# bolcom/serenade

Hardware: AMD Instinct MI355X
Metric: predict_next queries/sec (higher is better)
Workload: dtype u32 ids / i32 accumulators / f64 scores; 1 GPU; BASELINE configs[2]: synthetic 60000000 interactions / 1760000 items, k=1500 m=2500 idf_weighting=2 last_items=4 how_many=21; batch_per_gpu=1048576, query_pool_batches=2, parallelism=query-sharded replicas x1 (no data-path collective), index=csr (built by this library)

## Files before the change

serenade_amd/csrc/srn_fast.hip:

```cpp
#include <hip/hip_runtime.h>

#include <cstdio>
#include <cstdlib>

#include "srn_device.h"
#include "srn_prep.h"
#include "srn_kernels.h"

namespace srn {

#ifndef SRN_FAST_NT
#define SRN_FAST_NT 1
#endif
typedef uint32_t fin_v4u __attribute__((ext_vector_type(4)));
__device__ __forceinline__ void fin_store(uint4* p, const uint4& v) {
#if SRN_FAST_NT
    __builtin_nontemporal_store((fin_v4u{v.x, v.y, v.z, v.w}), reinterpret_cast<fin_v4u*>(p));
#else
    *p = v;
#endif
}
__device__ __forceinline__ uint4 fin_load(const uint4* p) {
#if SRN_FAST_NT
    const fin_v4u v = __builtin_nontemporal_load(reinterpret_cast<const fin_v4u*>(p)); return make_uint4(v.x, v.y, v.z, v.w);
#else
    return *p;
#endif
}
template <typename T> __device__ __forceinline__ void row_store(T* p, T v) {
#if SRN_FAST_NT
    __builtin_nontemporal_store(v, p);
#else
    *p = v;
#endif
}

enum { FS_NB = 0, FS_FAIL, FS_SURV, FS_CCNT, FS_HITS, FS_LIVE, FS_SCAN_A = 8, FS_SCAN_B = 8, FS_W3 = 8, FS_CLS = 16, FS_TACC = 32 };
static constexpr uint32_t F_SIDF = F_LDS_BYTES, F_SATTR = F_SIDF + 512 * 8, F_TOTAL = F_SATTR + 512, F_SINV = F_W10 + 384;
static_assert(F_TOTAL * F_WG_PER_CU <= 160 * 1024, "LDS budget with the sample constants");

#ifndef SRN_FAST_RELOAD_ROWS
#define SRN_FAST_RELOAD_ROWS 0
#endif
#ifndef SRN_FAST_PRIO_LEVELS
#define SRN_FAST_PRIO_LEVELS 22201333
#endif
enum { FP_REC = 10000000, FP_FRONT = 1000000, FP_CUT = 100000, FP_REQ = 10000, FP_WALK = 1000, FP_HARV = 100, FP_WB = 10, FP_HAND = 1 };
#ifndef SRN_FAST_PRIO_X
#define SRN_FAST_PRIO_X 92
#endif
#define FAST_PRIO_X(div) do { if (SRN_FAST_PRIO_LEVELS && ((SRN_FAST_PRIO_X) / (div)) % 10 != 9) __builtin_amdgcn_s_setprio((short)(((SRN_FAST_PRIO_X) / (div)) % 10)); } while (0)
#ifndef SRN_MID_PRIO_LEVELS
#define SRN_MID_PRIO_LEVELS SRN_FAST_PRIO_LEVELS
#endif
#define FAST_PRIO(ph) do { if (SRN_FAST_PRIO_LEVELS) __builtin_amdgcn_s_setprio((short)((((MID) ? (SRN_MID_PRIO_LEVELS) : (SRN_FAST_PRIO_LEVELS)) / (ph)) % 10)); } while (0)
#ifndef SRN_FAST_STOP
#define SRN_FAST_STOP (-1)
#endif
#ifndef SRN_FAST_TICK_TID
#define SRN_FAST_TICK_TID 0
#endif
#define FAST_TICK(ph) \
    do { if (ticking && tid == (SRN_FAST_TICK_TID)) { const long long t_ = clock64(); tacc[ph] += (unsigned long long)(t_ - t_prev); t_prev = t_; } } while (0); \
    if (SRN_FAST_STOP == (ph)) continue

__device__ __forceinline__ uint32_t fast_offset_of(uint32_t idx, uint64_t r) {
    if (idx < F_REP_ITEMS) return (F_DIRECT + idx * F_REP + ((uint32_t)r & (F_REP - 1u))) * 4u;
    return idx < F_DIRECT ? idx * 4u : (F_SKETCH - F_HOT) + (idx & (F_SK_WORDS - 1u)) * 4u;
}
#ifndef SRN_FAST_PHANTOM_OOR
#define SRN_FAST_PHANTOM_OOR 1
#endif
static constexpr uint32_t F_PHANTOM_WORDS = 256u;
static constexpr uint32_t F_PHANTOM = SRN_FAST_PHANTOM_OOR ? F_BIG_TOTAL - (F_TOTAL - F_SIDF) - 256u * 4u - F_M_MAX : F_DUMP;
static_assert(!SRN_FAST_PHANTOM_OOR || (F_PHANTOM >= F_TOTAL && F_PHANTOM % 4u == 0u), "the phantom words lie beyond the 53 KB forms' LDS allocation");
static_assert(F_PHANTOM + F_PHANTOM_WORDS * 4u - F_HOT <= 65536u, "16-bit row offsets");
static_assert(!SRN_FAST_PHANTOM_OOR || F_PHANTOM_WORDS * 4u <= F_M_MAX, "inside the numerator bytes' room");
__device__ __forceinline__ uint32_t fast_phantom(uint64_t r, uint32_t j) {
    return (F_PHANTOM - F_HOT) + ((((uint32_t)r * 0x9E3779B1u + j * 0x85EBCA6Bu) >> 21) & (F_PHANTOM_WORDS - 1u)) * 4u;
}
__global__ __launch_bounds__(1024) void rows_to_packed_kernel(const uint64_t* __restrict__ row_off, const uint32_t* __restrict__ row_items, uint64_t n,
                                                              const uint32_t* __restrict__ block_base, uint32_t* __restrict__ packed, uint32_t* __restrict__ ext16) {
    __shared__ uint32_t wave_tot[16];
    const uint64_t r = (uint64_t)blockIdx.x * 1024 + threadIdx.x;
    const int lane = threadIdx.x & 63, wave = threadIdx.x >> 6;
    uint64_t o = 0, len = 0;
    if (r < n) { o = row_off[r]; len = row_off[r + 1] - o; }
    const uint32_t e = len > 30 ? (uint32_t)((len - 28 + 7) / 8) : 0u;
    const uint32_t inc = wave_incl_scan(e);
    if (lane == 63) wave_tot[wave] = inc;
    __syncthreads();
    uint32_t base = block_base[blockIdx.x];
    for (int w = 0; w < wave; ++w) base += wave_tot[w];
    const uint32_t eblk = base + inc - e;
    if (r > n) return;
    const uint32_t inl = len > 30 ? 28u : (uint32_t)len;
    uint32_t sl[16];
    auto half = [&](uint32_t j) -> uint32_t { return j < inl ? fast_offset_of(row_items[o + j], r) : fast_phantom(r, j); };
    sl[0] = (uint32_t)(len > 0xFFFFu ? 0xFFFFu : len);
#pragma unroll
    for (uint32_t wd = 1; wd < 16; ++wd) sl[wd] = half(2 * wd - 2) | (half(2 * wd - 1) << 16);
    if (len > 30) {
        sl[15] = eblk;
        for (uint32_t b = 0; b < e; ++b) {
            uint32_t wv[4];
#pragma unroll
            for (uint32_t x = 0; x < 4; ++x) {
                const uint64_t j0 = 28 + 8ull * b + 2 * x;
                const uint32_t lo = j0 < len ? fast_offset_of(row_items[o + j0], r) : fast_phantom(r, (uint32_t)j0);
                const uint32_t hi = j0 + 1 < len ? fast_offset_of(row_items[o + j0 + 1], r) : fast_phantom(r, (uint32_t)j0 + 1);
                wv[x] = lo | (hi << 16);
            }
            reinterpret_cast<uint4*>(ext16)[(size_t)eblk + b] = make_uint4(wv[0], wv[1], wv[2], wv[3]);
        }
    }
    uint4* dst = reinterpret_cast<uint4*>(packed + r * 16);
#pragma unroll
// ... 213 lines not shown
        if (f.serve == nullptr) {
        if (alen) { if (tid < 8u) a_items[tid] = f.tiny_items[tid]; if (tid == 0u) { a_off[0] = 0u; a_off[1] = alen; } __syncthreads(); }
        if (tid < PREP_LANES) prep_group(ix_arg, alen ? (const uint64_t*)a_items : p.items_flat, alen ? (const uint32_t*)a_off : p.q_off, alen ? 0u : blockIdx.x, tid, p.m, p.max_len,
                                         const_cast<char*>(p.prep) + (size_t)blockIdx.x * p.prep_stride, nullptr, 0u, nullptr);
        __syncthreads();
        }
    }

    uint32_t* misc = (uint32_t*)(smem + F_MISC);
    uint8_t* wlut = (uint8_t*)(smem + F_WLUT);
    uint16_t* w10t = (uint16_t*)(smem + F_W10);
    uint32_t* nbl = (uint32_t*)(smem + F_NBL);
    unsigned long long* ckey = (unsigned long long*)(smem + F_CAND);
    uint32_t* cidx = (uint32_t*)(smem + F_CAND + F_CAND_CAP * 8);
    char* const acc_base = smem + F_HOT;
    uint32_t* hot = (uint32_t*)(smem + F_HOT);
    uint32_t* ikeys = (uint32_t*)(smem + F_TABLE);
    int* iacc = (int*)(smem + F_TABLE + F_TABLE_WORDS * 4);
    uint2* hits = (uint2*)(smem + F_HITS);
    uint32_t* surv = (uint32_t*)(smem + F_SURV);
    constexpr uint32_t SURV_CAP = F_SURV_WORDS - 256u;
    uint32_t* const cls_area = BIG ? (uint32_t*)(smem + SIDF) - 256 : surv + SURV_CAP;
    uint32_t* const dn_area = cls_area - F_M_MAX / 4u;
    uint2* const nb2 = reinterpret_cast<uint2*>(dn_area - F_K_MAX * 2u);
    uint32_t* thist = surv + SURV_CAP;
    auto num_of = [&](uint32_t set) -> uint32_t {
        if constexpr (MID) return (uint32_t)wlut[set & 31u] + (uint32_t)wlut[32u + (set >> 5)];
        else return (uint32_t)wlut[set]; };
    auto w10_of = [&](uint32_t set) -> uint32_t {
        if constexpr (MID) { const uint32_t lo = set & 31u, hi = set >> 5; const uint32_t mp = lo ? (uint32_t)wlut[64u + lo] : (uint32_t)wlut[96u + hi]; return (9u - mp) * ((uint32_t)wlut[lo] + (uint32_t)wlut[32u + hi]); }
        else return (uint32_t)w10t[set]; };

    unsigned long long* tacc = (unsigned long long*)(smem + F_MISC + FS_TACC * 4);
    if (tid < 16u) tacc[tid] = 0ull;
    const bool ticking = p.phase_cycles != nullptr;
    const bool business = (p.flags & SRN_FLAG_BUSINESS_LOGIC) != 0u;
    const uint32_t n_kept = ix.n_kept;
    auto qpos = [&](uint32_t pq) -> uint32_t { return ((wave + NW * (pq >> 6)) << 6) + (pq & 63u); };

    uint32_t* const pre = (uint32_t*)(smem + F_W10 + 64);
    bool have_pre = false;
    { const ItemMeta m0 = f.meta_sample[tid];
      ((double*)(smem + SIDF))[tid] = m0.idf > 0.0 ? m0.idf : 1.0; ((uint8_t*)(smem + SATTR))[tid] = (uint8_t)m0.attr;
      if (tid < 16u) ((double*)(smem + SINV))[tid] = tid < 8u ? f.inv_idf_hot[tid] : f.inv_idf_hi; }
    const bool listed = !MID && MODE == FM_BACK && f.mid_list != nullptr;
    const uint32_t q_end = TINY ? p.nq : LONG ? *f.long_cnt : BIG ? *f.bigq_cnt : MID || listed ? *f.mid_cnt : p.nq;
    const bool ordered = !MID && MODE != FM_FRONT && f.order != nullptr && !listed;
    const uint32_t ox = blockIdx.x & 7u;
    const bool serving = TINY && f.serve != nullptr;
    const uint32_t qi_step = serving ? 0u : ordered ? gridDim.x >> 3 : gridDim.x;
    uint32_t serve_seq = 0u; bool serve_have = false; unsigned long long serve_t0 = 0ull, serve_c0 = 0ull;
    if constexpr (TINY) { if (serving) serve_seq = __atomic_load_n(&(f.serve + blockIdx.x)->done_seq, __ATOMIC_RELAXED); }
    const uint32_t qi_end = ordered ? ord_count(f.order_dups != nullptr ? p.nq - *f.order_dups : p.nq, ox) : q_end;
    for (uint32_t qi = ordered ? blockIdx.x >> 3 : (MODE == FM_FRONT ? f.q_base : 0u) + blockIdx.x; qi < qi_end; qi += qi_step) {
        if constexpr (TINY) {
            if (serving) {
                uint32_t* const sv_flag = reinterpret_cast<uint32_t*>(smem + F_W10 + 64 + 192);
                unsigned long long* const sv_items = reinterpret_cast<unsigned long long*>(smem + F_W10 + 64); uint32_t* const sv_off = reinterpret_cast<uint32_t*>(smem + F_W10 + 64 + 128);
                ServeCtl* const c = f.serve + blockIdx.x;
                __syncthreads();
                if (wave == 0u) {
                    __threadfence_system();
                    uint32_t leave = 0u;
                    if (serve_have && lane == 0u) {
                        const uint32_t cnt = __atomic_load_n(&p.out_counts[blockIdx.x], __ATOMIC_RELAXED);
                        if (cnt & 0x80000000u) { (void)atomicExch(&f.slow_cnt[SC_GENERAL], 0u); (void)atomicExch(&f.slow_cnt[SC_MID], 0u); (void)atomicExch(&f.slow_cnt[SC_BIG_TICKET_LO], 0u); (void)atomicExch(&f.slow_cnt[SC_BIG_TICKET_HI], 0u); }
                        const unsigned long long t_end = wall_clock64();
                        c->stamp[2] = (uint32_t)(t_end - serve_t0); c->stamp[3] = (uint32_t)((unsigned long long)clock64() - serve_c0);
                        __atomic_store_n(&c->count, cnt, __ATOMIC_RELAXED);
                        __atomic_store_n(&c->status, (cnt & 0x80000000u) ? 1u : 0u, __ATOMIC_RELAXED);
                        __threadfence_system();
                        __atomic_store_n(&c->done_seq, serve_seq, __ATOMIC_RELAXED);
                    }
                    const unsigned long long t0 = wall_clock64(), idle = __builtin_nontemporal_load(&c->idle_ticks);
                    uint32_t w = 0u, s_new = 0u, n = 0u;
                    for (;;) {
                        if (lane < 16u) w = __atomic_load_n(reinterpret_cast<const uint32_t*>(c) + lane, __ATOMIC_RELAXED);
                        s_new = (uint32_t)__builtin_amdgcn_readlane((int)w, 0); n = min((uint32_t)__builtin_amdgcn_readlane((int)w, 1), 16u);
                        if (s_new != serve_seq) {
                            uint32_t x = lane >= 4u && lane < 4u + 2u * min(n, 5u) ? w : 0u;
#pragma unroll
                            for (int d = 1; d < 16; d <<= 1) x ^= __shfl_xor(x, d, 16);
                            if ((uint32_t)__builtin_amdgcn_readlane((int)x, 0) == ((uint32_t)__builtin_amdgcn_readlane((int)w, 2) ^ s_new ^ n)) break;
                        }
                        if ((uint32_t)__builtin_amdgcn_readlane((int)w, 3) != 0u || wall_clock64() - t0 > idle) { leave = 1u; break; }
                    }
                    if (!leave) {
                        serve_seq = s_new; serve_have = true; serve_t0 = wall_clock64(); serve_c0 = (unsigned long long)clock64();
                        if (lane >= 4u && lane < 14u) reinterpret_cast<uint32_t*>(sv_items)[lane - 4u] = w;
                        if (n > 5u && lane < 2u * (n - 5u)) reinterpret_cast<uint32_t*>(sv_items)[10u + lane] = __atomic_load_n(reinterpret_cast<const uint32_t*>(c->more) + lane, __ATOMIC_RELAXED);
                        if (lane == 0u) { sv_off[0] = 0u; sv_off[1] = n; p.out_counts[blockIdx.x] = 0x80000002u; c->stamp[0] = (uint32_t)(serve_t0 - t0); }
                    }
                    if (lane == 0u) sv_flag[0] = leave;
                }
                __syncthreads();
                if (sv_flag[0] != 0u) break;
                if (tid < PREP_LANES) prep_group(ix_arg, (const uint64_t*)sv_items, (const uint32_t*)sv_off, 0u, tid, p.m, p.max_len, const_cast<char*>(p.prep) + (size_t)blockIdx.x * p.prep_stride, nullptr, 0u, nullptr);
                __syncthreads();
                if (tid == 0u) c->stamp[1] = (uint32_t)(wall_clock64() - serve_t0);
            }
        }
        const uint32_t q = TINY ? qi : LONG ? f.long_list[qi] : BIG ? f.bigq_list[qi] : MID || listed ? f.mid_list[qi] : ordered ? (uint32_t)f.order[ord_pos(ox, qi)] : qi;
        const uint32_t q_ord_next = ordered && qi + qi_step < qi_end ? (uint32_t)f.order[ord_pos(ox, qi + qi_step)]
                                  : listed && qi + qi_step < qi_end ? f.mid_list[qi + qi_step] : 0xFFFFFFFFu;
#ifndef SRN_MID_PREFETCH
#define SRN_MID_PREFETCH 0
#endif
        const uint32_t q_after = !(MID && SRN_MID_PREFETCH) ? 0xFFFFFFFFu : qi + gridDim.x < q_end ? (BIG ? f.bigq_list : f.mid_list)[qi + gridDim.x] : 0xFFFFFFFFu;
        long long t_prev = ticking ? clock64() : 0;
        FAST_PRIO(FP_REC);
        const char* const rec = p.prep + (size_t)q * p.prep_stride;
        struct { uint32_t U, rmax, xlo, sumw, L, n_staged, cur_attr, unsafe; } hd;
        constexpr uint32_t HW = (uint32_t)sizeof(PrepHead) / 4u;
        struct { uint32_t idx, kept; unsigned long long base; } x0{kNone, 0u, 0ull};
        if (have_pre) {
            auto uni = [&](uint32_t w) -> uint32_t { return (uint32_t)__builtin_amdgcn_readfirstlane((int)pre[w]); };
            hd.U = uni(0); hd.rmax = uni(1); hd.xlo = uni(2); hd.sumw = uni(3); hd.L = uni(6); hd.n_staged = uni(7); hd.cur_attr = uni(16); hd.unsafe = uni(17);
            if (lane < (LONG ? 32u : MID ? 16u : 8u) && lane < hd.L) { const uint32_t* it = pre + HW + 6u * lane; x0.idx = it[0]; x0.kept = it[3]; x0.base = ((unsigned long long)it[5] << 32) | it[4]; }
        } else {
            const PrepHead h0 = *(const PrepHead*)rec;
            hd.U = h0.U; hd.rmax = h0.rmax; hd.xlo = h0.xlo; hd.sumw = h0.sumw; hd.L = h0.L; hd.n_staged = h0.n_staged; hd.cur_attr = h0.cur_attr; hd.unsafe = h0.unsafe;
            if ((MID ? lane < (LONG ? 32u : 16u) && lane < p.max_len : lane < 8u) && lane < hd.L) { const PrepItem pi = ((const PrepItem*)(rec + sizeof(PrepHead)))[lane]; x0.idx = pi.idx; x0.kept = pi.kept; x0.base = pi.base; }
        }
        have_pre = false;
        const uint32_t L = hd.L, n = hd.n_staged, U = hd.U;
        unsigned long long rm = __ballot(x0.kept > 0u);
#ifdef SRN_FAST_EXP_ONELIST
        rm &= 0ull - rm;
#endif
        const uint32_t nr = (uint32_t)__popcll(rm);
        const bool rel = MID || (WIDE && nr > 3u);
        const uint32_t NB = LONG ? F_LONG_NB : MID ? max(nr, 4u) : WIDE && !rel ? 3u : 4u, NBM = (1u << NB) - 1u, base = rel ? hd.xlo : 0u;
        const bool fits = hd.unsafe != 0u ? false : LONG ? L >= 1u && L <= F_LONG_LMAX && L <= p.max_len && hd.sumw <= F_LONG_CLASSES && nr <= F_LONG_LISTS && 2u * n + 8u + F_LONG_RES_WORDS <= MW && hd.rmax - hd.xlo < (1u << (32u - F_LONG_NB))
                        : MID ? L >= 1u && L <= F_MID_LMAX && L <= p.max_len && hd.sumw <= F_MID_CLASSES && nr <= F_MID_LISTS && 2u * n + 8u + 256u <= MW && hd.rmax - hd.xlo < (1u << (32u - NB))
                              : L >= 1u && L <= 8u && L <= p.max_len && hd.sumw <= 15u && nr <= 4u && 2u * n + 8u <= MW && (!rel || hd.rmax - hd.xlo < (1u << 28));
        uint32_t* const xq = MODE == FM_FUSED ? nullptr : f.xchg + (size_t)q * f.xchg_stride;
        if (!fits) {
            if constexpr (MODE == FM_FRONT) { if (tid == 0) xq[0] = 0xFFFFFFFFu; }
            else if (tid == 0) {
                if (hd.unsafe != 0u) f.slow_list[atomicAdd(&f.slow_cnt[SC_GENERAL], 1u)] = q;
                else if (!MID && MODE == FM_FUSED && f.bigq_list != nullptr && L >= 1u && L <= 8u && L <= p.max_len && hd.sumw <= 15u && nr <= 4u && hd.rmax - hd.xlo < (1u << 28) &&
                    2u * n + 8u + 256u <= (F_BIG_TOTAL - (F_TOTAL - F_SIDF) - F_WORK) / 4u) f.bigq_list[atomicAdd(f.bigq_cnt, 1u)] = q;
                else if (!MID && MODE == FM_FUSED && f.mid_list != nullptr && L >= 1u && L <= F_MID_LMAX && L <= p.max_len) f.mid_list[atomicAdd(f.mid_cnt, 1u)] = q;
                else if (!MID && MODE == FM_FUSED && f.long_list != nullptr && L > F_MID_LMAX && L <= F_LONG_LMAX && L <= p.max_len) f.long_list[atomicAdd(f.long_cnt, 1u)] = q;
                else if (MID && !BIG && f.bigq_list != nullptr && L >= 1u && L <= F_MID_LMAX && L <= p.max_len && hd.sumw <= F_MID_CLASSES && nr <= F_MID_LISTS && hd.rmax - hd.xlo < (1u << (32u - NB)) &&
                         2u * n + 8u + 256u <= (F_BIG_TOTAL - (F_TOTAL - F_SIDF) - F_WORK) / 4u) f.bigq_list[atomicAdd(f.bigq_cnt, 1u)] = q;
                else f.slow_list[atomicAdd(&f.slow_cnt[SC_GENERAL], 1u)] = q;
            }
            continue;
        }
        if (n == 0u) { if (tid == 0) { if constexpr (MODE == FM_FRONT) xq[0] = 0u; else p.out_counts[q] = 0u; } continue; }
        uint32_t kp[NL], ps[NL]; const uint32_t* src[NL];
#pragma unroll
        for (int r = 0; r < NL; ++r) {
            const int l = rm ? __ffsll((long long)rm) - 1 : 0;
            kp[r] = rm ? (uint32_t)__builtin_amdgcn_readlane((int)x0.kept, l) : 0u;
            const uint32_t blo = (uint32_t)__builtin_amdgcn_readlane((int)(uint32_t)x0.base, l), bhi = (uint32_t)__builtin_amdgcn_readlane((int)(uint32_t)(x0.base >> 32), l);
            src[r] = ix.post_rank + (((unsigned long long)bhi << 32) | blo);
            ps[r] = (uint32_t)l;
            rm &= rm - 1ull;
        }
        const uint32_t cur_idx = (uint32_t)__builtin_amdgcn_readlane((int)x0.idx, 0);
        const uint32_t cur_attr = hd.cur_attr;
        const uint32_t s1 = kp[0], s2 = s1 + kp[1], s3 = s2 + kp[2];

        uint32_t v[4][5];
        uint32_t K = 0;
        uint32_t pfv[4] = {0u, 0u, 0u, 0u};
        uint32_t xsv[3] = {0u, 0u, 0u};
        if constexpr (MODE == FM_BACK) {
            const uint32_t kv = xq[0];
#pragma unroll
            for (int t = 0; t < 3; ++t) xsv[t] = xq[1u + min(wave * 64u + lane + (uint32_t)t * BLOCK, f.xchg_stride - 2u)];
            K = (uint32_t)__builtin_amdgcn_readfirstlane((int)kv);
        } else {
#pragma unroll
        for (int r = 0; r < 4; ++r)
#pragma unroll
            for (int j = 0; j < 5; ++j) { v[r][j] = 0u; if ((uint32_t)j * BLOCK < kp[r]) v[r][j] = src[r][min(tid + j * BLOCK, kp[r] - 1u)]; }
        }
        __syncthreads();
        FAST_PRIO(FP_FRONT);
        if constexpr (MODE != FM_BACK) {
#pragma unroll
        for (int r = 0; r < 4; ++r)
#pragma unroll
            for (int j = 0; j < 5; ++j) asm volatile("" : "+v"(v[r][j]));
        }
        FAST_TICK(0);
        if (tid < (uint32_t)FS_TACC) misc[tid] = 0;
#ifndef SRN_FAST_EARLY_CLEAR
#define SRN_FAST_EARLY_CLEAR 0
#endif
        const uint32_t clr_lo = (!SRN_FAST_EARLY_CLEAR || MODE == FM_FRONT) ? F_TABLE : (MODE == FM_BACK || nr <= 1u) ? F_HOT : min(F_TABLE, max(F_HOT, (F_WORK + (2u * n + 16u) * 4u + 15u) & ~15u));
        if (SRN_FAST_EARLY_CLEAR && MODE != FM_FRONT) {
            uint4* z = reinterpret_cast<uint4*>(smem);
            for (uint32_t i = clr_lo / 16u + tid; i < F_TABLE / 16u; i += BLOCK) z[i] = make_uint4(0u, 0u, 0u, 0u);
        }
        if constexpr (LONG) {
            if (tid < 32u) {
                uint32_t pr = 0u;
#pragma unroll
                for (int r = 0; r < NL; ++r) pr = tid == (uint32_t)(31 - r) ? ps[r] : pr;
                wlut[tid] = (uint8_t)(L - pr); wlut[32u + tid] = (uint8_t)pr;
            }
        } else
        if constexpr (MID) {
            if (tid < 64u) {
                const uint32_t half = tid >> 5, hs = tid & 31u;
                uint32_t num = 0u, mp = 0u;
                const uint32_t lo = hs ? (uint32_t)__ffs((int)hs) - 1u : 0u;
#pragma unroll
                for (int r = 0; r < 5; ++r) { const uint32_t pr = half ? ps[5 + r] : ps[r]; num += ((hs >> r) & 1u) ? L - pr : 0u; mp = lo == (uint32_t)r ? pr : mp; }
                wlut[tid] = (uint8_t)num; wlut[64u + tid] = (uint8_t)mp;
            }
        } else
        if (tid < (1u << nr)) {
            const uint32_t num = ((tid & 1u) ? L - ps[0] : 0u) + ((tid & 2u) ? L - ps[1] : 0u) + ((tid & 4u) ? L - ps[2] : 0u) + ((tid & 8u) ? L - ps[3] : 0u);
            const uint32_t lo = tid ? (uint32_t)__ffs((int)tid) - 1u : 0u;
            const uint32_t mp = lo == 0u ? ps[0] : lo == 1u ? ps[1] : lo == 2u ? ps[2] : ps[3];
            wlut[tid] = (uint8_t)num; w10t[tid] = (uint16_t)((9u - mp) * num);
        }
        if constexpr (MODE == FM_BACK) {
            if (K == 0xFFFFFFFFu) { if (tid == 0) f.slow_list[atomicAdd(&f.slow_cnt[SC_GENERAL], 1u)] = q; continue; }
            if (K == 0u) { if (tid == 0) p.out_counts[q] = 0u; continue; }
        } else
        if (nr == 1u) {
            K = min(kp[0], p.k);
#pragma unroll
            for (int j = 0; j < 3; ++j) { const uint32_t e = tid + j * BLOCK; if ((uint32_t)j * BLOCK < K && e < K) {
                if constexpr (LONG) nb2[e] = make_uint2(((v[0][j] - base) << NB) | 31u, (uint32_t)((9 - (int)ps[0]) * (int)(L - ps[0])));
                else nbl[e] = ((v[0][j] - base) << NB) | 1u; } }
            __syncthreads();
            FAST_TICK(1);
        } else {
        uint32_t* const B1 = (uint32_t*)(smem + F_WORK); uint32_t* const B0 = B1 + n;
        static_assert(F_WORK == F_NBL, "the m-cut writes the neighbour list in place");
        if constexpr (MID) {
            const uint32_t nlev = nr <= 2u ? 1u : nr <= 4u ? 2u : nr <= 8u ? 3u : nr <= 16u ? 4u : 5u;
            uint32_t* const X = (nlev & 1u) ? B1 : B0; uint32_t* const Y = (nlev & 1u) ? B0 : B1;
            uint32_t pre_r[NL];
// ... 199 lines not shown
        }
        }
        }

        FAST_TICK(4);
        if constexpr (SRN_FAST_ROW_PREFETCH == 2 && !MID && MODE == FM_FUSED && !FRAG) asm volatile("" :: "v"(pfv[0]), "v"(pfv[1]), "v"(pfv[2]), "v"(pfv[3]));
        FAST_PRIO(FP_REQ); FAST_PRIO_X(10);
        if constexpr (MODE == FM_FRONT) {
            if (tid == 0) xq[0] = K;
#pragma unroll
            for (int j = 0; j < 3; ++j) { const uint32_t e = tid + (uint32_t)j * BLOCK; if ((uint32_t)j * BLOCK < K && e < K) xq[1u + e] = nbl[e]; }
            continue;
        }

        uint32_t svr[3]; uint4 rq[3], rq1[3];
        uint32_t wvr[3] = {0u, 0u, 0u};
#pragma unroll
        for (int t = 0; t < 3; ++t) {
            const uint32_t j = wave * 64u + lane + (uint32_t)t * BLOCK;
            if constexpr (MODE == FM_BACK) svr[t] = j < K ? xsv[t] : 0u;
            else if constexpr (LONG) { const uint2 e2 = nb2[K ? min(j, K - 1u) : 0u]; svr[t] = K ? e2.x : 0u; wvr[t] = e2.y; }
            else
            svr[t] = K ? nbl[min(j, K - 1u)] : 0u;
            const size_t r = (MODE == FM_BACK ? j < K : K != 0u) ? (size_t)(base + (svr[t] >> NB)) : (size_t)n_kept;
            rq[t] = *reinterpret_cast<const uint4*>(&f.row_packed[r * (FRAG ? 1 : 4)]); rq1[t] = make_uint4(0u, 0u, 0u, 0u);
        }
        if (((SRN_FAST_PRIO_X) / 10) % 10 != 9) FAST_PRIO(FP_REQ);
        {
            uint4* z = reinterpret_cast<uint4*>(smem + F_HOT);
            for (uint32_t i = tid; i < (clr_lo - F_HOT) / 16u; i += BLOCK) z[i] = make_uint4(0u, 0u, 0u, 0u);
            if (tid < 64u) reinterpret_cast<uint4*>(thist)[tid] = make_uint4(0u, 0u, 0u, 0u);
            if (tid < F_TABLE_WORDS / 4u) { reinterpret_cast<uint4*>(ikeys)[tid] = make_uint4(EMPTY32, EMPTY32, EMPTY32, EMPTY32);
                                            reinterpret_cast<uint4*>(iacc)[tid] = make_uint4(0u, 0u, 0u, 0u); }
        }
        __syncthreads();
        FAST_PRIO(FP_WALK);
        FAST_TICK(8);
        auto add2 = [&](uint32_t wd, uint32_t w) {
            if constexpr (LONG) {
                const bool neg = (int)w < 0; const uint32_t a = wd & 0xFFFFu, b = wd >> 16;
                if (!neg || a < F_SKETCH - F_HOT) atomicAdd((uint32_t*)(acc_base + a), w);
                if (!neg || b < F_SKETCH - F_HOT) atomicAdd((uint32_t*)(acc_base + b), w);
            } else {
            atomicAdd((uint32_t*)(acc_base + (wd & 0xFFFFu)), w); atomicAdd((uint32_t*)(acc_base + (wd >> 16)), w); } };
        constexpr uint32_t INL1 = FRAG ? 6u : 14u, INL2 = FRAG ? 20u : 28u;
        uint32_t cnt3 = 0;
#pragma unroll
        for (int t = 0; t < 3; ++t) {
            const bool m3 = wave * 64u + lane + (uint32_t)t * BLOCK < K && (rq[t].x & 0xFFFFu) > INL1;
            const unsigned long long b3 = __ballot(m3);
            if (m3) nbl[qpos(cnt3 + (uint32_t)__popcll(b3 & lt))] = LONG ? wave * 64u + lane + (uint32_t)t * BLOCK : svr[t];
            cnt3 += (uint32_t)__popcll(b3);
        }
#ifdef SRN_FAST_SUBTICKS
        FAST_TICK(5);
#endif
        uint32_t wr[3];
#pragma unroll
        for (int t = 0; t < 3; ++t) wr[t] = LONG ? wvr[t] : w10_of(svr[t] & NBM);
        if constexpr (!FRAG) {
#pragma unroll
            for (int t = 0; t < 3; ++t) {
                const bool more6 = wave * 64u + lane + (uint32_t)t * BLOCK < K && (rq[t].x & 0xFFFFu) > 6u;
                const size_t r1 = more6 ? (size_t)(base + (svr[t] >> NB)) : (size_t)n_kept;
                rq1[t] = *reinterpret_cast<const uint4*>(&f.row_packed[r1 * 4 + 1]);
            }
        }
        auto tok_slot = [&](uint32_t tok) -> uint32_t { if constexpr (LONG) return nb2[tok].x; else return tok; };
        auto tok_w = [&](uint32_t tok, uint32_t slot) -> uint32_t { if constexpr (LONG) return nb2[tok].y; else return w10_of(slot & NBM); };
        auto q3_load = [&](uint32_t p0, uint32_t& tok, uint32_t& sv, uint32_t& hdr, uint4& c4, uint4& d4, uint32_t& blk) {
            tok = nbl[qpos(min(p0 + lane, cnt3 - 1u))];
            sv = tok_slot(tok);
            if constexpr (FRAG) {
                const uint4 s4 = *reinterpret_cast<const uint4*>(f.row_packed + (size_t)(base + (sv >> NB)));
                hdr = s4.x;
                const uint4* eb = reinterpret_cast<const uint4*>(f.row_ext16) + ((hdr & 0xFFFFu) > 6u ? (size_t)s4.w : (size_t)0);
                c4 = eb[0]; d4 = eb[1]; blk = s4.w + 2u;
            } else {
                const RowQuad* rowp = f.row_packed + (size_t)(base + (sv >> NB)) * 4;
                hdr = *reinterpret_cast<const uint32_t*>(rowp); c4 = *reinterpret_cast<const uint4*>(rowp + 2); d4 = *reinterpret_cast<const uint4*>(rowp + 3); blk = 0u;
            } };
        uint32_t tk3 = 0, sv3 = 0, hdr3 = 0, blk3 = 0; uint4 c43 = make_uint4(0u, 0u, 0u, 0u), d43 = c43;
        if (cnt3) q3_load(0u, tk3, sv3, hdr3, c43, d43, blk3);
        const uint32_t w3 = cnt3 ? tok_w(tk3, sv3) : 0u;
        const uint32_t qn = MID ? q_after : ordered || listed ? q_ord_next : q + gridDim.x;
        const bool park = MID ? q_after != 0xFFFFFFFFu : ordered || listed ? q_ord_next != 0xFFFFFFFFu : qn < p.nq;
        if (wave == 1u && park) {
            const char* const rn = p.prep + (size_t)qn * p.prep_stride + lane * 4u;
            const uint32_t dst = (uint32_t)__builtin_amdgcn_readfirstlane((int)lds_addr(pre));
            if (lane * 4u < p.prep_stride) glds_dword_uncounted(rn, dst);
            if (256u + lane * 4u < min(p.prep_stride, 320u)) glds_dword_uncounted(rn + 256, dst + 256u);
        }
#pragma unroll
        for (int t = 0; t < 3; ++t) {
            if (wave * 64u + (uint32_t)t * BLOCK < K) {
                const bool act = wave * 64u + lane + (uint32_t)t * BLOCK < K;
                const uint32_t w = wr[t], len = rq[t].x & 0xFFFFu;
                if constexpr (FRAG) { if (act) { add2(rq[t].y, w); add2(rq[t].z, w); if (len <= 6u) add2(rq[t].w, w); } }
                else if (act) { add2(rq[t].y, w); add2(rq[t].z, w); add2(rq[t].w, w); }
            }
        }
        if constexpr (!FRAG) {
#pragma unroll
        for (int t = 0; t < 3; ++t) {
            if (wave * 64u + (uint32_t)t * BLOCK < K) {
                const bool act = wave * 64u + lane + (uint32_t)t * BLOCK < K;
                const uint32_t w = wr[t], len = rq[t].x & 0xFFFFu;
                if (act && len > 6u) { add2(rq1[t].x, w); add2(rq1[t].y, w); add2(rq1[t].z, w); add2(rq1[t].w, w); }
            }
        }
        }
        auto add_tail = [&](uint32_t p0, uint32_t w, uint32_t hdr, const uint4& c4, const uint4& d4, uint32_t blk) {
            const bool act = p0 + lane < cnt3;
            const uint32_t len = hdr & 0xFFFFu;
            const bool more = FRAG ? true : len > 30u;
            if constexpr (FRAG) {
                if (act) { add2(c4.x, w); add2(c4.y, w); add2(c4.z, w); add2(c4.w, w); }
                if (act && len > 12u) { add2(d4.x, w); add2(d4.y, w); add2(d4.z, w); add2(d4.w, w); }
            } else if (act) {
                add2(c4.x, w); add2(c4.y, w); add2(c4.z, w); add2(c4.w, w);
                add2(d4.x, w); add2(d4.y, w); add2(d4.z, w);
                if (len <= 30u) add2(d4.w, w);
            }
            for (uint32_t t8 = INL2; __ballot(act && more && t8 < len) != 0ull; t8 += 8u) {
                if (act && more && t8 < len) {
                    const uint4 e4 = reinterpret_cast<const uint4*>(f.row_ext16)[(size_t)blk + ((t8 - INL2) >> 3)];
                    add2(e4.x, w); add2(e4.y, w); add2(e4.z, w); add2(e4.w, w);
                }
            } };
#ifdef SRN_FAST_SUBTICKS
        FAST_TICK(6);
#endif
        FAST_PRIO_X(1);
        { fin_v4u dv = {d43.x, d43.y, d43.z, d43.w};
          asm volatile("" : "+v"(hdr3), "+v"(dv));
          d43 = make_uint4(dv.x, dv.y, dv.z, dv.w); }
        if constexpr (!FRAG) blk3 = d43.w;
        if (cnt3) add_tail(0u, w3, hdr3, c43, d43, blk3);
        for (uint32_t p0 = 64u; p0 < cnt3; p0 += 64u) { uint32_t tk, sv, hdr, blk; uint4 c4, d4; q3_load(p0, tk, sv, hdr, c4, d4, blk); if constexpr (!FRAG) blk = d4.w; add_tail(p0, tok_w(tk, sv), hdr, c4, d4, blk); }
#ifdef SRN_FAST_SUBTICKS
        FAST_TICK(7);
#endif
        __syncthreads();
        FAST_PRIO(FP_HARV);
        FAST_TICK(9);
        uint32_t t32m1; uint32_t floor_b;
        {
            const uint32_t e = lane * NW + wave;
            uint32_t v = hot[e];
            if (F_REP_ITEMS && e < F_REP_ITEMS) {
                const uint4* rp = reinterpret_cast<const uint4*>(hot + F_DIRECT + e * F_REP);
                const uint4 a = rp[0], b = rp[1];
                v = a.x + a.y + a.z + a.w + b.x + b.y + b.z + b.w;
            }
            if (!SRN_FAST_PHANTOM_OOR || BIG)
            for (uint32_t i = tid; i < F_PHANTOM_WORDS; i += BLOCK) ((uint32_t*)(smem + F_PHANTOM))[i] = 0u;
            bool valid = (LONG ? (int)v > 0 : v != 0u) && e != cur_idx;
            double x = 0.0; uint32_t tie = 0;
            tie = f.meta_sample[tid].id_rank;
            if (business) valid = valid && business_ok(cur_attr, (uint32_t)((const uint8_t*)(smem + SATTR))[tid]);
            if (valid) x = ((const double*)(smem + SIDF))[tid] * (double)v;
            const uint32_t k32 = (uint32_t)((unsigned long long)__double_as_longlong(x) >> 32);
            {
                uint32_t vv = k32, third = 0;
#pragma unroll
                for (int t = 0; t < 3; ++t) {
                    const uint32_t mx = wave_max(vv);
                    third = mx;
                    const unsigned long long bal = __ballot(vv == mx);
                    if ((int)lane == __ffsll((long long)bal) - 1) vv = 0;
                }
                for (uint32_t t = 3u; t < ((p.how_many + 7u) >> 3); ++t) {
                    const uint32_t mx = wave_max(vv);
                    third = mx;
                    const unsigned long long bal = __ballot(vv == mx);
                    if ((int)lane == __ffsll((long long)bal) - 1) vv = 0;
                }
                if (lane == 0u) misc[FS_W3 + wave] = third;
            }
            __syncthreads();
            uint32_t t32 = 0xFFFFFFFFu;
#pragma unroll
            for (int w = 0; w < NW; ++w) t32 = min(t32, misc[FS_W3 + w]);
            t32m1 = t32 ? t32 - 1u : 0u;
            const bool take = valid && k32 >= t32m1;
            const uint32_t at = wave_append(take, &misc[FS_CCNT]);
            if (take) { if (at < F_CAND_CAP) { ckey[at] = (unsigned long long)__double_as_longlong(x); cidx[at] = tie; } else misc[FS_FAIL] = 1;
                        const uint32_t hb = k32 >> 16, tb = t32 >> 16; if (t32) atomicAdd(&thist[hb > tb ? min(hb - tb, 255u) : 0u], 1u); }
            const double x_lo = __longlong_as_double((long long)((unsigned long long)t32m1 << 32));
            const double inv = ((const double*)(smem + SINV))[min(lane, 8u)];
            const uint32_t my_floor = (uint32_t)fmin(4.0e9, fmax(1.0, floor(x_lo * inv * (1.0 - 1e-9)) - 1.0));
            floor_b = (uint32_t)__builtin_amdgcn_readlane((int)my_floor, 8);
            {
                const uint32_t wv = (uint32_t)__builtin_amdgcn_readfirstlane((int)wave);
                const uint4* h4 = reinterpret_cast<const uint4*>(hot);
                static_assert(F_HOT_WORDS == 4096 || F_HOT_WORDS == 3840, "quads per thread below (3840: the 40 KB timing experiment)");
                constexpr uint32_t NQ2 = F_HOT_WORDS / 4u - 128u - (uint32_t)BLOCK;
                const uint4 a4 = h4[128u + tid];
                const uint4 b4 = tid < NQ2 ? h4[128u + (uint32_t)BLOCK + tid] : make_uint4(0u, 0u, 0u, 0u);
                if (tid == NQ2 - 1u) hot[F_HOT_WORDS - 1u] = 0u;
                const uint32_t fl1 = (uint32_t)__builtin_amdgcn_readlane((int)my_floor, (int)(1u + (wv >> 1)));
                const uint32_t fl2 = (uint32_t)__builtin_amdgcn_readlane((int)my_floor, (int)min(5u + (wv >> 1), 7u));
                auto quad = [&](const uint4& q4, uint32_t e0, uint32_t fl) {
                    const uint32_t mx = LONG ? (uint32_t)max(max(max((int)q4.x, (int)q4.y), max((int)q4.z, (int)q4.w)), 0) : max(max(q4.x, q4.y), max(q4.z, q4.w));
                    if (__ballot(mx >= fl) == 0ull) return;
                    const uint32_t vv[4] = {q4.x, q4.y, q4.z, q4.w};
#pragma unroll
                    for (uint32_t j = 0; j < 4u; ++j) {
                        const uint32_t e2 = e0 + j;
                        const bool pass = (LONG ? (int)vv[j] >= (int)fl : vv[j] >= fl) && e2 != cur_idx && e2 < F_DIRECT;
                        const uint32_t at2 = wave_append(pass, &misc[FS_SURV]);
                        if (pass) { if (at2 < SURV_CAP && vv[j] < (1u << 20)) surv[at2] = (e2 << 20) | vv[j]; else atomicOr(&misc[FS_FAIL], 2u); }
                    } };
                quad(a4, 512u + 4u * tid, fl1);
                quad(b4, 512u + 4u * ((uint32_t)BLOCK + tid), fl2);
            }
        }
        __syncthreads();
        {
            const uint4 h4 = reinterpret_cast<const uint4*>(thist)[lane];
            const uint32_t sum4 = h4.x + h4.y + h4.z + h4.w, pre = wave_incl_scan(sum4);
            uint32_t above = (uint32_t)__builtin_amdgcn_readlane((int)pre, 63) - pre;
            const uint32_t need = p.how_many;
            const bool mine = above < need && need <= above + sum4;
            uint32_t bin = 4u * lane + 3u;
            if (above + h4.w < need) { above += h4.w; bin = 4u * lane + 2u;
                if (above + h4.z < need) { above += h4.z; bin = 4u * lane + 1u;
                    if (above + h4.y < need) bin = 4u * lane; } }
            const unsigned long long mb = __ballot(mine);
            const uint32_t bsel = mb ? (uint32_t)__builtin_amdgcn_readlane((int)bin, __ffsll((long long)mb) - 1) : 0u;
            if (bsel) {
                const uint32_t t32b = (((t32m1 + 1u) >> 16) + bsel) << 16;
                t32m1 = t32b - 1u;
// ... 6 lines not shown
        FAST_PRIO(FP_WB);
        {
            const uint32_t ns = min(misc[FS_SURV], SURV_CAP);
            for (uint32_t i = tid; i < ns; i += BLOCK) {
                const uint32_t sv = surv[i], e = sv >> 20, v = sv & 0xFFFFFu;
                const ItemMeta mt = ix.meta[e];
                const double x = (mt.idf > 0.0 ? mt.idf : 1.0) * (double)v;
                const bool take = (uint32_t)((unsigned long long)__double_as_longlong(x) >> 32) >= t32m1 && (!business || business_ok(cur_attr, mt.attr));
                const uint32_t at = wave_append(take, &misc[FS_CCNT]);
                if (take) { if (at < F_CAND_CAP) { ckey[at] = (unsigned long long)__double_as_longlong(x); cidx[at] = mt.id_rank; } else misc[FS_FAIL] = 1; }
            }
        }
        {
            const uint4* sk4 = reinterpret_cast<const uint4*>(smem + F_SKETCH);
            uint32_t mx = 0;
            for (uint32_t i = tid; i < F_SK_WORDS / 4u; i += BLOCK) { const uint4 w4 = sk4[i]; mx = max(max(mx, w4.x), max(max(w4.y, w4.z), w4.w)); }
            if (__ballot(mx >= floor_b) != 0ull && lane == 0u) misc[FS_LIVE] = 1u;
        }
        __syncthreads();
        have_pre = park;
        const bool live = misc[FS_LIVE] != 0u;
        if (live) {
        {
            uint32_t dbg_hits = 0;
            auto chk2 = [&](uint32_t hm, uint32_t wd) -> uint32_t {
                const uint32_t a = *(const uint32_t*)(acc_base + max(wd & 0xFFFFu, F_ZERO_OFF)), b = *(const uint32_t*)(acc_base + max(wd >> 16, F_ZERO_OFF));
                return (hm << 2) | (a >= floor_b ? 2u : 0u) | (b >= floor_b ? 1u : 0u); };
            auto list_hits = [&](uint32_t hm, uint32_t npos, uint32_t sv, uint32_t j0) {
                const uint32_t c = (uint32_t)__popc(hm);
                if (__ballot(c != 0u) == 0ull) return;
                dbg_hits += c;
                const uint32_t inc = wave_incl_scan(c);
                uint32_t base = 0; if (lane == 63u) base = atomicAdd(&misc[FS_HITS], inc);
                uint32_t at = (uint32_t)__builtin_amdgcn_readlane((int)base, 63) + inc - c;
                while (hm) {
                    const uint32_t b = 31u - (uint32_t)__clz((int)hm); hm &= ~(1u << b);
                    if (at < F_HIT_CAP) hits[at] = make_uint2(sv, j0 + (npos - 1u - b)); else atomicOr(&misc[FS_FAIL], 4u);
                    ++at;
                }
            };
            auto mx2 = [&](uint32_t mx, uint32_t wd) -> uint32_t {
                const uint32_t a = *(const uint32_t*)(acc_base + max(wd & 0xFFFFu, F_ZERO_OFF)), b = *(const uint32_t*)(acc_base + max(wd >> 16, F_ZERO_OFF));
                return max(max(mx, a), b); };
            uint32_t tk3b = 0, sv3b = 0, hdr3b = 0, blk3b = 0; uint4 c43b = make_uint4(0u, 0u, 0u, 0u), d43b = c43b;
#if SRN_FAST_RELOAD_ROWS
#pragma unroll
            for (int t = 0; t < 3; ++t) {
                const size_t r = K ? (size_t)(base + (svr[t] >> NB)) : (size_t)n_kept;
                rq[t] = *reinterpret_cast<const uint4*>(&f.row_packed[r * 4]);
                rq1[t] = *reinterpret_cast<const uint4*>(&f.row_packed[r * 4 + 1]);
            }
#endif
            if (cnt3) q3_load(0u, tk3b, sv3b, hdr3b, c43b, d43b, blk3b);
            if constexpr (!FRAG) blk3b = d43b.w;
#pragma unroll
            for (int t = 0; t < 3; ++t) {
                if (wave * 64u + (uint32_t)t * BLOCK < K) {
                    const bool act = wave * 64u + lane + (uint32_t)t * BLOCK < K, two = (rq[t].x & 0xFFFFu) > 6u;
                    uint32_t mx = 0;
                    if constexpr (FRAG) {
                        if (act) { mx = mx2(mx2(0u, rq[t].y), rq[t].z); if (!two) mx = mx2(mx, rq[t].w); }
                        if (__ballot(mx >= floor_b) != 0ull) {
                            uint32_t hm = 0;
                            if (act) { hm = chk2(chk2(0u, rq[t].y), rq[t].z); hm = two ? hm << 2 : chk2(hm, rq[t].w); }
                            list_hits(hm, 6u, LONG ? wave * 64u + lane + (uint32_t)t * BLOCK : svr[t], 0u);
                        }
                    } else {
                    if (act) { mx = mx2(mx2(mx2(0u, rq[t].y), rq[t].z), rq[t].w); if (two) mx = mx2(mx2(mx2(mx2(mx, rq1[t].x), rq1[t].y), rq1[t].z), rq1[t].w); }
                    if (__ballot(mx >= floor_b) != 0ull) {
                        uint32_t hm = 0;
                        if (act) {
                            hm = chk2(chk2(chk2(0u, rq[t].y), rq[t].z), rq[t].w) << 8;
                            if (two) hm = chk2(chk2(chk2(chk2(hm >> 8, rq1[t].x), rq1[t].y), rq1[t].z), rq1[t].w);
                        }
                        list_hits(hm, 14u, LONG ? wave * 64u + lane + (uint32_t)t * BLOCK : svr[t], 0u);
                    }
                    }
                }
            }
            auto chk_tail = [&](uint32_t p0, uint32_t sv, uint32_t hdr, const uint4& c4, const uint4& d4, uint32_t blk) {
                const bool act = p0 + lane < cnt3;
                const uint32_t len = hdr & 0xFFFFu;
                const bool more = FRAG ? true : len > 30u;
                uint32_t hm = 0, mx = 0;
                if constexpr (FRAG) {
                    const bool two = len > 12u;
                    if (act) { mx = mx2(mx2(mx2(mx2(0u, c4.x), c4.y), c4.z), c4.w); if (two) mx = mx2(mx2(mx2(mx2(mx, d4.x), d4.y), d4.z), d4.w); }
                    if (__ballot(mx >= floor_b) != 0ull) {
                        uint32_t hmd = 0;
                        if (act) { hm = chk2(chk2(chk2(chk2(0u, c4.x), c4.y), c4.z), c4.w); if (two) hmd = chk2(chk2(chk2(chk2(0u, d4.x), d4.y), d4.z), d4.w); }
                        list_hits(hm, 8u, sv, 4u); list_hits(hmd, 8u, sv, 12u);
                    }
                } else {
                if (act) { mx = mx2(mx2(mx2(mx2(mx2(mx2(mx2(0u, c4.x), c4.y), c4.z), c4.w), d4.x), d4.y), d4.z); if (len <= 30u) mx = mx2(mx, d4.w); }
                if (__ballot(mx >= floor_b) != 0ull) {
                if (act) {
                    hm = chk2(chk2(chk2(chk2(chk2(chk2(chk2(0u, c4.x), c4.y), c4.z), c4.w), d4.x), d4.y), d4.z);
                    if (len > 30u) hm <<= 2; else hm = chk2(hm, d4.w);
                }
                list_hits(hm, 16u, sv, 14u); }
                }
                for (uint32_t t8 = INL2; __ballot(act && more && t8 < len) != 0ull; t8 += 8u) {
                    uint32_t hm2 = 0;
                    if (act && more && t8 < len) {
                        const uint4 e4 = reinterpret_cast<const uint4*>(f.row_ext16)[(size_t)blk + ((t8 - INL2) >> 3)];
                        hm2 = chk2(chk2(chk2(chk2(0u, e4.x), e4.y), e4.z), e4.w);
                    }
                    list_hits(hm2, 8u, sv, t8);
                } };
            if (cnt3) chk_tail(0u, tk3b, hdr3b, c43b, d43b, blk3b);
            for (uint32_t p0 = 64u; p0 < cnt3; p0 += 64u) { uint32_t tk, sv, hdr, blk; uint4 c4, d4; q3_load(p0, tk, sv, hdr, c4, d4, blk); if constexpr (!FRAG) blk = d4.w; chk_tail(p0, tk, hdr, c4, d4, blk); }
            if (ticking) { const uint32_t hs = wave_sum(dbg_hits); if (lane == 0u && hs) atomicAdd(&tacc[5], (unsigned long long)hs); }
        }
        __syncthreads();
        FAST_TICK(11);
        {
            const uint32_t nh = min(misc[FS_HITS], F_HIT_CAP);
            if (ticking && tid == 0 && nh == 0u) tacc[7] += 1ull;
            bool ovf = false;
            for (uint32_t i = tid; i < nh; i += BLOCK) {
                const uint2 h = hits[i];
                const uint32_t hslot = tok_slot(h.x);
                const uint32_t* os = reinterpret_cast<const uint32_t*>(ix.row_slots + (size_t)(base + (hslot >> NB)) * (FRAG ? 1 : 4));
                const uint32_t len = os[0], j = h.y;
                uint32_t it = EMPTY32;
                if constexpr (FRAG) { if (j < len) it = len <= 3u ? os[1 + j] : (j < 2u ? os[2 + j] : ix.row_ext[os[1] + (j - 2u)]); }
                else
                if (j < len) it = len <= 15u ? os[1 + j] : (j < 14u ? os[2 + j] : ix.row_ext[os[1] + (j - 14u)]);
                if (business && it != EMPTY32 && it >= F_DIRECT && !business_ok(cur_attr, ix.meta[it].attr)) it = EMPTY32;
                if (it != EMPTY32 && it >= F_DIRECT && item_insert(ikeys, iacc, F_TABLE_BUCKETS, it, (int)tok_w(h.x, hslot)) < 0) ovf = true;
            }
            if (ovf) atomicOr(&misc[FS_FAIL], 8u);
        }
        __syncthreads();
        }
        FAST_TICK(12);
        if (misc[FS_FAIL]) {
            if (tid == 0) { f.slow_list[atomicAdd(&f.slow_cnt[SC_GENERAL], 1u)] = q; if (ticking) { const uint32_t c = misc[FS_FAIL]; tacc[15] += (c & 1u) + ((unsigned long long)((c >> 1) & 1u) << 16) + ((unsigned long long)((c >> 2) & 1u) << 32) + ((unsigned long long)((c >> 3) & 1u) << 48); } }
            continue;
        }
        if (wave != 0u) continue;
        FAST_PRIO(FP_HAND);
        uint32_t ln = lane; asm volatile("" : "+v"(ln));
        const unsigned long long ltl = (1ull << ln) - 1ull;
        uint2* tl = hits;
        uint32_t nt = 0;
        if (live)
#pragma unroll
        for (uint32_t b0 = 0; b0 < (F_TABLE_BUCKETS + 63u) / 64u; ++b0) {
            const uint32_t bk = b0 * 64u + ln;
            uint4 kq = make_uint4(EMPTY32, EMPTY32, EMPTY32, EMPTY32), aq = make_uint4(0u, 0u, 0u, 0u);
            if (bk < F_TABLE_BUCKETS) { kq = reinterpret_cast<const uint4*>(ikeys)[bk]; aq = reinterpret_cast<const uint4*>(iacc)[bk]; }
            const uint32_t kk[4] = {kq.x, kq.y, kq.z, kq.w}, aa[4] = {aq.x, aq.y, aq.z, aq.w};
#pragma unroll
            for (int s4 = 0; s4 < 4; ++s4) {
                const bool in = kk[s4] != EMPTY32 && kk[s4] != cur_idx && (LONG ? (int)aa[s4] >= (int)floor_b : aa[s4] >= floor_b);
                const unsigned long long bm = __ballot(in);
                if (in) tl[nt + (uint32_t)__popcll(bm & ltl)] = make_uint2(kk[s4], aa[s4]);
                nt += (uint32_t)__popcll(bm);
            }
        }
        uint32_t cnt = misc[FS_CCNT];
        if (cnt + nt > F_FIN_ENTRIES && cnt <= F_CAND_CAP) {
            unsigned long long xs[3]; uint32_t ti[3];
// ... 346 lines not shown
```

Measured before the change: 56.57 million queries/s.

## Carry next query id across iterations and pin loads with scalar broadcasts

The next query id from the order or mid list is now loaded through a scalar-held base pointer. It is issued before the block barrier and carried into the next iteration as a wave-uniform value, so the dependent lookup no longer sits at the top of each loop. The prep header words are broadcast with readfirstlane into scalar registers, and empty asm barriers pin when the tail-check loads arrive, to shape the compiler's wait placement. It also adds configurable debug subtick macros. The risk is extra register pressure, and the compiler-scheduling hints may not help.

```diff
diff --git a/serenade_amd/csrc/srn_fast.hip b/serenade_amd/csrc/srn_fast.hip
--- a/serenade_amd/csrc/srn_fast.hip
+++ b/serenade_amd/csrc/srn_fast.hip
@@ -63,6 +63,16 @@
 #define FAST_TICK(ph) \
     do { if (ticking && tid == (SRN_FAST_TICK_TID)) { const long long t_ = clock64(); tacc[ph] += (unsigned long long)(t_ - t_prev); t_prev = t_; } } while (0); \
     if (SRN_FAST_STOP == (ph)) continue
+#if defined(SRN_FAST_SUBTICKS) && SRN_FAST_SUBTICKS == 2
+#define FAST_SUBTICK_P0(ph) FAST_TICK(ph)
+#define FAST_SUBTICK_WA(ph) do { } while (0)
+#elif defined(SRN_FAST_SUBTICKS)
+#define FAST_SUBTICK_P0(ph) do { } while (0)
+#define FAST_SUBTICK_WA(ph) FAST_TICK(ph)
+#else
+#define FAST_SUBTICK_P0(ph) do { } while (0)
+#define FAST_SUBTICK_WA(ph) do { } while (0)
+#endif
 
 __device__ __forceinline__ uint32_t fast_offset_of(uint32_t idx, uint64_t r) {
     if (idx < F_REP_ITEMS) return (F_DIRECT + idx * F_REP + ((uint32_t)r & (F_REP - 1u))) * 4u;
@@ -382,7 +392,16 @@
     uint32_t serve_seq = 0u; bool serve_have = false; unsigned long long serve_t0 = 0ull, serve_c0 = 0ull;
     if constexpr (TINY) { if (serving) serve_seq = __atomic_load_n(&(f.serve + blockIdx.x)->done_seq, __ATOMIC_RELAXED); }
     const uint32_t qi_end = ordered ? ord_count(f.order_dups != nullptr ? p.nq - *f.order_dups : p.nq, ox) : q_end;
-    for (uint32_t qi = ordered ? blockIdx.x >> 3 : (MODE == FM_FRONT ? f.q_base : 0u) + blockIdx.x; qi < qi_end; qi += qi_step) {
+    const bool carried = !TINY && !MID && (ordered || listed);
+    unsigned long long ent_base = (unsigned long long)(uintptr_t)(ordered ? (const void*)f.order : (const void*)f.mid_list);
+    asm volatile("" : "+s"(ent_base));
+    auto entry_at = [&](uint32_t i) -> uint32_t {
+        typedef __attribute__((address_space(1))) const uint32_t glb_u32;
+        return *(glb_u32*)(uintptr_t)(ent_base + (ordered ? (unsigned long long)ord_pos(ox, i) << 3 : (unsigned long long)i << 2)); };
+    const uint32_t qi_first = ordered ? blockIdx.x >> 3 : (MODE == FM_FRONT ? f.q_base : 0u) + blockIdx.x;
+    uint32_t q_carry = 0xFFFFFFFFu;
+    if (carried && qi_first < qi_end) q_carry = (uint32_t)__builtin_amdgcn_readfirstlane((int)entry_at(qi_first));
+    for (uint32_t qi = qi_first; qi < qi_end; qi += qi_step) {
         if constexpr (TINY) {
             if (serving) {
                 uint32_t* const sv_flag = reinterpret_cast<uint32_t*>(smem + F_W10 + 64 + 192);
@@ -430,15 +449,15 @@
                 if (tid == 0u) c->stamp[1] = (uint32_t)(wall_clock64() - serve_t0);
             }
         }
-        const uint32_t q = TINY ? qi : LONG ? f.long_list[qi] : BIG ? f.bigq_list[qi] : MID || listed ? f.mid_list[qi] : ordered ? (uint32_t)f.order[ord_pos(ox, qi)] : qi;
-        const uint32_t q_ord_next = ordered && qi + qi_step < qi_end ? (uint32_t)f.order[ord_pos(ox, qi + qi_step)]
-                                  : listed && qi + qi_step < qi_end ? f.mid_list[qi + qi_step] : 0xFFFFFFFFu;
+        const uint32_t q = TINY ? qi : LONG ? f.long_list[qi] : BIG ? f.bigq_list[qi] : MID ? f.mid_list[qi] : carried ? q_carry : qi;
+        auto next_entry = [&]() -> uint32_t { return carried && qi + qi_step < qi_end ? entry_at(qi + qi_step) : 0xFFFFFFFFu; };
 #ifndef SRN_MID_PREFETCH
 #define SRN_MID_PREFETCH 0
 #endif
         const uint32_t q_after = !(MID && SRN_MID_PREFETCH) ? 0xFFFFFFFFu : qi + gridDim.x < q_end ? (BIG ? f.bigq_list : f.mid_list)[qi + gridDim.x] : 0xFFFFFFFFu;
         long long t_prev = ticking ? clock64() : 0;
         FAST_PRIO(FP_REC);
+        FAST_SUBTICK_P0(5);
         const char* const rec = p.prep + (size_t)q * p.prep_stride;
         struct { uint32_t U, rmax, xlo, sumw, L, n_staged, cur_attr, unsafe; } hd;
         constexpr uint32_t HW = (uint32_t)sizeof(PrepHead) / 4u;
@@ -449,8 +468,12 @@
             if (lane < (LONG ? 32u : MID ? 16u : 8u) && lane < hd.L) { const uint32_t* it = pre + HW + 6u * lane; x0.idx = it[0]; x0.kept = it[3]; x0.base = ((unsigned long long)it[5] << 32) | it[4]; }
         } else {
             const PrepHead h0 = *(const PrepHead*)rec;
-            hd.U = h0.U; hd.rmax = h0.rmax; hd.xlo = h0.xlo; hd.sumw = h0.sumw; hd.L = h0.L; hd.n_staged = h0.n_staged; hd.cur_attr = h0.cur_attr; hd.unsafe = h0.unsafe;
+            uint32_t hw[8] = {h0.U, h0.rmax, h0.xlo, h0.sumw, h0.L, h0.n_staged, h0.cur_attr, h0.unsafe};
+            asm volatile("" : "+v"(hw[0]), "+v"(hw[1]), "+v"(hw[2]), "+v"(hw[3]), "+v"(hw[4]), "+v"(hw[5]), "+v"(hw[6]), "+v"(hw[7]));
+            auto sc = [&](uint32_t w) -> uint32_t { return (uint32_t)__builtin_amdgcn_readfirstlane((int)w); };
+            hd.U = sc(hw[0]); hd.rmax = sc(hw[1]); hd.xlo = sc(hw[2]); hd.sumw = sc(hw[3]); hd.L = sc(hw[4]); hd.n_staged = sc(hw[5]); hd.cur_attr = sc(hw[6]); hd.unsafe = sc(hw[7]);
             if ((MID ? lane < (LONG ? 32u : 16u) && lane < p.max_len : lane < 8u) && lane < hd.L) { const PrepItem pi = ((const PrepItem*)(rec + sizeof(PrepHead)))[lane]; x0.idx = pi.idx; x0.kept = pi.kept; x0.base = pi.base; }
+            asm volatile("" : "+v"(x0.idx));
         }
         have_pre = false;
         const uint32_t L = hd.L, n = hd.n_staged, U = hd.U;
@@ -477,9 +500,10 @@
                          2u * n + 8u + 256u <= (F_BIG_TOTAL - (F_TOTAL - F_SIDF) - F_WORK) / 4u) f.bigq_list[atomicAdd(f.bigq_cnt, 1u)] = q;
                 else f.slow_list[atomicAdd(&f.slow_cnt[SC_GENERAL], 1u)] = q;
             }
+            q_carry = (uint32_t)__builtin_amdgcn_readfirstlane((int)next_entry());
             continue;
         }
-        if (n == 0u) { if (tid == 0) { if constexpr (MODE == FM_FRONT) xq[0] = 0u; else p.out_counts[q] = 0u; } continue; }
+        if (n == 0u) { if (tid == 0) { if constexpr (MODE == FM_FRONT) xq[0] = 0u; else p.out_counts[q] = 0u; } q_carry = (uint32_t)__builtin_amdgcn_readfirstlane((int)next_entry()); continue; }
         uint32_t kp[NL], ps[NL]; const uint32_t* src[NL];
 #pragma unroll
         for (int r = 0; r < NL; ++r) {
@@ -509,7 +533,10 @@
 #pragma unroll
             for (int j = 0; j < 5; ++j) { v[r][j] = 0u; if ((uint32_t)j * BLOCK < kp[r]) v[r][j] = src[r][min(tid + j * BLOCK, kp[r] - 1u)]; }
         }
+        const uint32_t q_next_v = next_entry();
+        FAST_SUBTICK_P0(6);
         __syncthreads();
+        FAST_SUBTICK_P0(7);
         FAST_PRIO(FP_FRONT);
         if constexpr (MODE != FM_BACK) {
 #pragma unroll
@@ -517,6 +544,8 @@
 #pragma unroll
             for (int j = 0; j < 5; ++j) asm volatile("" : "+v"(v[r][j]));
         }
+        q_carry = (uint32_t)__builtin_amdgcn_readfirstlane((int)q_next_v);
+        const uint32_t q_ord_next = q_carry;
         FAST_TICK(0);
         if (tid < (uint32_t)FS_TACC) misc[tid] = 0;
 #ifndef SRN_FAST_EARLY_CLEAR
@@ -822,9 +851,7 @@
             if (m3) nbl[qpos(cnt3 + (uint32_t)__popcll(b3 & lt))] = LONG ? wave * 64u + lane + (uint32_t)t * BLOCK : svr[t];
             cnt3 += (uint32_t)__popcll(b3);
         }
-#ifdef SRN_FAST_SUBTICKS
-        FAST_TICK(5);
-#endif
+        FAST_SUBTICK_WA(5);
         uint32_t wr[3];
 #pragma unroll
         for (int t = 0; t < 3; ++t) wr[t] = LONG ? wvr[t] : w10_of(svr[t] & NBM);
@@ -898,9 +925,7 @@
                     add2(e4.x, w); add2(e4.y, w); add2(e4.z, w); add2(e4.w, w);
                 }
             } };
-#ifdef SRN_FAST_SUBTICKS
-        FAST_TICK(6);
-#endif
+        FAST_SUBTICK_WA(6);
         FAST_PRIO_X(1);
         { fin_v4u dv = {d43.x, d43.y, d43.z, d43.w};
           asm volatile("" : "+v"(hdr3), "+v"(dv));
@@ -908,9 +933,7 @@
         if constexpr (!FRAG) blk3 = d43.w;
         if (cnt3) add_tail(0u, w3, hdr3, c43, d43, blk3);
         for (uint32_t p0 = 64u; p0 < cnt3; p0 += 64u) { uint32_t tk, sv, hdr, blk; uint4 c4, d4; q3_load(p0, tk, sv, hdr, c4, d4, blk); if constexpr (!FRAG) blk = d4.w; add_tail(p0, tok_w(tk, sv), hdr, c4, d4, blk); }
-#ifdef SRN_FAST_SUBTICKS
-        FAST_TICK(7);
-#endif
+        FAST_SUBTICK_WA(7);
         __syncthreads();
         FAST_PRIO(FP_HARV);
         FAST_TICK(9);
@@ -949,6 +972,7 @@
                 if (lane == 0u) misc[FS_W3 + wave] = third;
             }
             __syncthreads();
+            asm volatile("" : "+v"(tie));
             uint32_t t32 = 0xFFFFFFFFu;
 #pragma unroll
             for (int w = 0; w < NW; ++w) t32 = min(t32, misc[FS_W3 + w]);
@@ -1061,7 +1085,6 @@
             }
 #endif
             if (cnt3) q3_load(0u, tk3b, sv3b, hdr3b, c43b, d43b, blk3b);
-            if constexpr (!FRAG) blk3b = d43b.w;
 #pragma unroll
             for (int t = 0; t < 3; ++t) {
                 if (wave * 64u + (uint32_t)t * BLOCK < K) {
@@ -1117,8 +1140,14 @@
                     }
                     list_hits(hm2, 8u, sv, t8);
                 } };
+            auto arrived = [&](uint32_t& hdr, uint4& c4, uint4& d4) {
+                fin_v4u cv = {c4.x, c4.y, c4.z, c4.w}, dv = {d4.x, d4.y, d4.z, d4.w};
+                asm volatile("" : "+v"(hdr), "+v"(cv), "+v"(dv));
+                c4 = make_uint4(cv.x, cv.y, cv.z, cv.w); d4 = make_uint4(dv.x, dv.y, dv.z, dv.w); };
+            arrived(hdr3b, c43b, d43b);
+            if constexpr (!FRAG) blk3b = d43b.w;
             if (cnt3) chk_tail(0u, tk3b, hdr3b, c43b, d43b, blk3b);
-            for (uint32_t p0 = 64u; p0 < cnt3; p0 += 64u) { uint32_t tk, sv, hdr, blk; uint4 c4, d4; q3_load(p0, tk, sv, hdr, c4, d4, blk); if constexpr (!FRAG) blk = d4.w; chk_tail(p0, tk, hdr, c4, d4, blk); }
+            for (uint32_t p0 = 64u; p0 < cnt3; p0 += 64u) { uint32_t tk, sv, hdr, blk; uint4 c4, d4; q3_load(p0, tk, sv, hdr, c4, d4, blk); arrived(hdr, c4, d4); if constexpr (!FRAG) blk = d4.w; chk_tail(p0, tk, hdr, c4, d4, blk); }
             if (ticking) { const uint32_t hs = wave_sum(dbg_hits); if (lane == 0u && hs) atomicAdd(&tacc[5], (unsigned long long)hs); }
         }
         __syncthreads();
```

New measurement: 56.78 million queries/s (median of 6 runs). No clear change (+0.4%).
